# ZENGXH/DMM_Net

Hardware: AMD Instinct MI355X
Metric: frames/sec (cost+match layer) at N=50 proposals, M=10 templates, 255x255 (higher is better)
Workload: dtype f32

## Files before the change

### dmm_net_amd/csrc/dmm_api.hip

```cpp
#include <limits.h>
#include <stdlib.h>

#include <atomic>

#include "dmm_launchers.h"
#include "dmm_solve.h"

namespace dmm {
static thread_local int g_last_hip_error = 0;
void set_last_hip_error(int e) { g_last_hip_error = e; }
static std::atomic<long long> g_launches{0};
void note_launch() { g_launches.fetch_add(1, std::memory_order_relaxed); }

static constexpr int kOptDefaults[DMM_OPT_COUNT] = {
     -1,       8,    -1,   0,
     0,      8192,         512,  512,
     1,           3,             320000,     2,
     128,        3,              512,  1,
     65,    1,           4,     1,
     -1,        1,    -1,  1,
};
static std::atomic<int> g_opts[DMM_OPT_COUNT] = {
    {kOptDefaults[0]},  {kOptDefaults[1]},  {kOptDefaults[2]},  {kOptDefaults[3]},  {kOptDefaults[4]},
    {kOptDefaults[5]},  {kOptDefaults[6]},  {kOptDefaults[7]},  {kOptDefaults[8]},  {kOptDefaults[9]},
    {kOptDefaults[10]}, {kOptDefaults[11]}, {kOptDefaults[12]}, {kOptDefaults[13]}, {kOptDefaults[14]},
    {kOptDefaults[15]}, {kOptDefaults[16]}, {kOptDefaults[17]}, {kOptDefaults[18]}, {kOptDefaults[19]},
    {kOptDefaults[20]}, {kOptDefaults[21]}, {kOptDefaults[22]}, {kOptDefaults[23]},
};
static_assert(DMM_OPT_COUNT == 24, "kOptDefaults / g_opts list every option");
int opt(int key) { return g_opts[key].load(std::memory_order_relaxed); }

static inline size_t align_up(size_t v, size_t a) { return (v + a - 1) / a * a; }

struct Workspace {
    int32_t *inter, *area_p, *area_t;
    float *featn_p, *featn_t, *cosv, *sim, *Rb;
    float *wide;
    size_t bytes;
};

static bool wide_shape(int N, int M) {
    const int Pp = N > M ? N : M + 1;
    return M > DMM_MAX_TEMPLATES || Pp > DMM_MAX_PROPOSALS || opt(DMM_OPT_FORCE_WIDE) == 1;
}

static Workspace carve(void *base, int B, int N, int M, int D) {
    const int Pp = N > M ? N : M + 1;
    Workspace w;
    size_t off = 0;
    auto take = [&](size_t n) {
        void *p = base ? (void *)((char *)base + off) : nullptr;
        off += align_up(n, 256);
        return p;
    };
    w.inter = (int32_t *)take(sizeof(int32_t) * ((size_t)B * M * N + (size_t)B * N + (size_t)B * M));
    w.area_p = w.inter ? w.inter + (size_t)B * M * N : nullptr;
    w.area_t = w.area_p ? w.area_p + (size_t)B * N : nullptr;
    w.featn_p = (float *)take(sizeof(float) * (size_t)B * N * D);
    w.featn_t = (float *)take(sizeof(float) * (size_t)B * M * D);
    w.cosv = (float *)take(sizeof(float) * (size_t)B * M * N);
    w.sim = (float *)take(sizeof(float) * (size_t)B * M * N);
    w.Rb = (float *)take(sizeof(float) * (size_t)B * M * Pp);
    w.wide = nullptr;
    if (wide_shape(N, M))
        w.wide = (float *)take(sizeof(float) * (size_t)B * wide_scratch_floats(M, Pp));
    w.bytes = off;
    return w;
}

static float *or_ws(float *out, float *ws) { return out ? out : ws; }

static Front ws_front(const Workspace &w, const void *masks_p, const void *masks_t, int dtype, int64_t sp_b, int64_t sp_n,
                      int64_t st_b, int64_t st_m, const float *feat_p, const float *feat_t, int B, int N, int M, int HW, int D,
                      const int32_t *n_valid, const int32_t *m_valid) {
    Front f{};
    f.masks_p = masks_p; f.masks_t = masks_t; f.dtype = dtype;
    f.sp_b = sp_b; f.sp_n = sp_n; f.st_b = st_b; f.st_m = st_m;
    f.feat_p = feat_p; f.feat_t = feat_t;
    f.B = B; f.N = N; f.M = M; f.HW = HW; f.D = D;
    f.n_valid = n_valid; f.m_valid = m_valid;
    f.cos = w.cosv;
    f.inter = w.inter; f.area_p = w.area_p; f.area_t = w.area_t;
    f.table_words = (size_t)B * M * N + (size_t)B * N + (size_t)B * M;
    f.featn_p = w.featn_p; f.featn_t = w.featn_t;
    return f;
}
static Front packed_front(const Workspace &w, const uint64_t *packed_p, int64_t pk_b, int64_t pk_n, const uint64_t *packed_t,
                          const float *feat_p, const float *feat_t, int B, int N, int M, int HW, int D,
                          const int32_t *n_valid, const int32_t *m_valid) {
    const int64_t wd = dmm_pack_words(HW);
    Front f = ws_front(w, packed_p, packed_t, DMM_PACKED1, pk_b, pk_n, (int64_t)M * wd, wd, feat_p, feat_t, B, N, M, HW, D,
                       n_valid, m_valid);
    f.ragged_lanes = true;
    return f;
}
}

extern "C" int dmm_abi_version(void) { return DMM_ABI_VERSION; }

extern "C" int dmm_set_option(int option, int value) {
    if (option < 0 || option >= DMM_OPT_COUNT) return DMM_ERR_BAD_ARG;
    switch (option) {
        case DMM_OPT_FEAT_BWD_FRAME: if (value < -1 || value > 2) return DMM_ERR_BAD_ARG; break;
        case DMM_OPT_COST_KERNEL: case DMM_OPT_SOLVER_KERNEL: case DMM_OPT_MIX_SHARED:
            if (value < -1 || value > 1) return DMM_ERR_BAD_ARG; break;
        case DMM_OPT_MIX_XCD: if (value < 0 || value > 7) return DMM_ERR_BAD_ARG; break;
        case DMM_OPT_FORCE_WIDE: case DMM_OPT_COSINE_KERNEL: case DMM_OPT_COST_XCD:
        case DMM_OPT_NMS_WAVE: case DMM_OPT_SMALL_FUSED: case DMM_OPT_MIX_SHARED_LOCKSTEP:
            if (value < 0 || value > 1) return DMM_ERR_BAD_ARG; break;
        case DMM_OPT_MIX_ALIGN: if (value != 16 && value != 32 && value != 64 && value != 128) return DMM_ERR_BAD_ARG; break;
        case DMM_OPT_MIX_NT: if (value < 0 || value > 3) return DMM_ERR_BAD_ARG; break;
        case DMM_OPT_COST_WGS: case DMM_OPT_COST_SMALL_WGS: case DMM_OPT_COST_TL_WGS: case DMM_OPT_MIX_WGS:
        case DMM_OPT_MIX_STEPQ: case DMM_OPT_GEMM_TUNE: case DMM_OPT_COS_ROWS_MIN_N: case DMM_OPT_MIX_SHARED_STEPS:
            if (value < 1) return DMM_ERR_BAD_ARG; break;
        default: if (value < 0) return DMM_ERR_BAD_ARG; break;
    }
    dmm::g_opts[option].store(value, std::memory_order_relaxed);
    return DMM_OK;
}

extern "C" int dmm_get_option(int option) {
    return (option < 0 || option >= DMM_OPT_COUNT) ? INT_MIN : dmm::opt(option);
}

extern "C" int dmm_reset_options(void) {
    for (int k = 0; k < DMM_OPT_COUNT; ++k) dmm::g_opts[k].store(dmm::kOptDefaults[k], std::memory_order_relaxed);
    return DMM_OK;
}

extern "C" const char *dmm_status_string(int status) {
    switch (status) {
        case DMM_OK: return "ok";
        case DMM_ERR_BAD_ARG: return "bad argument";
        case DMM_ERR_UNSUPPORTED: return "shape outside the compiled kernel envelope";
        case DMM_ERR_LAUNCH: return "HIP launch/runtime error (see dmm_last_hip_error)";
        case DMM_ERR_WORKSPACE: return "workspace too small";
        default: return "unknown status";
    }
}

extern "C" int dmm_last_hip_error(void) { return dmm::g_last_hip_error; }

extern "C" long long dmm_launch_count(void) { return dmm::g_launches.load(std::memory_order_relaxed); }

#define DMM_STR_(x) #x
#define DMM_STR(x) DMM_STR_(x)
extern "C" const char *dmm_build_info(void) { return "libdmm_match gfx950 (CDNA4, wave64) abi " DMM_STR(DMM_ABI_VERSION); }

extern "C" size_t dmm_workspace_bytes(int B, int N, int M, int D) {
    if (B <= 0 || N <= 0 || M <= 0 || D < 0) return 0;
    return dmm::carve(nullptr, B, N, M, D).bytes;
}

extern "C" int dmm_match_forward(const void *masks_p, const void *masks_t, int mask_dtype, const float *feat_p,
                                 const float *feat_t, const float *score_p, int B, int N, int M, int HW, int D,
                                 int64_t sp_b, int64_t sp_n, int64_t st_b, int64_t st_m, const int32_t *n_valid,
                                 const int32_t *m_valid, float score_weight, int max_iter, int proj_iter, float lr,
                                 int is_test, float *full_outmask, float *match_score, float *det_score,
                                 float *sim_out, float *R_out, float *Rb_out, int32_t *iters_out, void *workspace,
                                 size_t workspace_bytes, dmm_stream_t stream) {
    return dmm_match_forward_ws(masks_p, masks_t, mask_dtype, feat_p, feat_t, score_p, B, N, M, HW, D, sp_b, sp_n, st_b, st_m,
                                n_valid, m_valid, score_weight, max_iter, proj_iter, lr, is_test, full_outmask, match_score,
                                det_score, sim_out, R_out, Rb_out, iters_out, workspace, workspace_bytes, nullptr, stream);
}

extern "C" int dmm_match_forward_ws(const void *masks_p, const void *masks_t, int mask_dtype, const float *feat_p,
                                    const float *feat_t, const float *score_p, int B, int N, int M, int HW, int D,
                                    int64_t sp_b, int64_t sp_n, int64_t st_b, int64_t st_m, const int32_t *n_valid,
                                    const int32_t *m_valid, float score_weight, int max_iter, int proj_iter, float lr,
                                    int is_test, float *full_outmask, float *match_score, float *det_score,
                                    float *sim_out, float *R_out, float *Rb_out, int32_t *iters_out, void *workspace,
                                    size_t workspace_bytes, int *ws_state, dmm_stream_t stream) {
    const bool tables_zero = ws_state && *ws_state == DMM_WS_TABLES_ZERO;
    if (ws_state) *ws_state = DMM_WS_UNKNOWN;
    bool go;
    int rc = dmm::one_call_check(B, N, M, HW, D, masks_p && masks_t && feat_p && feat_t && score_p && full_outmask &&
                                 match_score && det_score && workspace, &go);
    if (!go) return rc;
    if (!dmm::soft_planes(mask_dtype)) return DMM_ERR_BAD_ARG;
    const dmm::Workspace w = dmm::carve(workspace, B, N, M, D);
    if (workspace_bytes < w.bytes) return DMM_ERR_WORKSPACE;
    const dmm::SolveIn in{w.cosv, w.inter, w.area_p, w.area_t, score_p, B, N, M, n_valid, m_valid};
    const dmm::SolveOut out{dmm::or_ws(sim_out, w.sim), R_out, dmm::or_ws(Rb_out, w.Rb), match_score, det_score, iters_out,
                            nullptr};
    const dmm::RelaxParams prm{max_iter, proj_iter, lr};
    if (dmm::wide_shape(N, M)) {
        if (!w.wide || B > 65535) return DMM_ERR_UNSUPPORTED;
// ... 120 lines not shown
```

### dmm_net_amd/csrc/dmm_gemm.hip

```cpp
#include <hipblaslt/hipblaslt.h>

#include <initializer_list>
#include <map>
#include <mutex>
#include <tuple>
#include <vector>

#include "dmm_common.h"

namespace dmm {
namespace {

struct GemmPlan {
    hipblasLtMatmulDesc_t desc = nullptr;
    hipblasLtMatrixLayout_t a = nullptr, b = nullptr, c = nullptr, d = nullptr;
    hipblasLtMatmulAlgo_t algo;
    size_t workspace = 0;
    bool ok = false;
    std::vector<hipblasLtMatmulHeuristicResult_t> candidates;
};

constexpr int kTuneCandidates = 24, kTuneRuns = 8;

std::mutex g_mu;
std::map<int, hipblasLtHandle_t> g_handles;
hipblasLtHandle_t handle_of(int dev) {
    auto it = g_handles.find(dev);
    if (it != g_handles.end()) return it->second;
    hipblasLtHandle_t h = nullptr;
    if (hipblasLtCreate(&h) != HIPBLAS_STATUS_SUCCESS) return nullptr;
    g_handles[dev] = h;
    return h;
}
std::map<std::tuple<int, int64_t, int, int, int, int, int>, GemmPlan> g_plans;

void release_plan(GemmPlan &p) {
    if (p.desc) hipblasLtMatmulDescDestroy(p.desc);
    for (hipblasLtMatrixLayout_t l : {p.a, p.b, p.c, p.d})
        if (l) hipblasLtMatrixLayoutDestroy(l);
    p = GemmPlan();
}

#define DMM_LT_TRY(expr)                                    \
    do {                                                    \
        if ((expr) != HIPBLAS_STATUS_SUCCESS) return false; \
    } while (0)

bool build_plan(hipblasLtHandle_t g_handle, GemmPlan &p, int64_t rows, int cin, int cout, bool relu, bool residual, size_t ws_limit) {
    const hipDataType bf16 = HIP_R_16BF;
    DMM_LT_TRY(hipblasLtMatmulDescCreate(&p.desc, HIPBLAS_COMPUTE_32F, HIP_R_32F));
    const hipblasOperation_t op_n = HIPBLAS_OP_N;
    DMM_LT_TRY(hipblasLtMatmulDescSetAttribute(p.desc, HIPBLASLT_MATMUL_DESC_TRANSA, &op_n, sizeof(op_n)));
    DMM_LT_TRY(hipblasLtMatmulDescSetAttribute(p.desc, HIPBLASLT_MATMUL_DESC_TRANSB, &op_n, sizeof(op_n)));
    const hipblasLtEpilogue_t epi = relu ? HIPBLASLT_EPILOGUE_RELU_BIAS : HIPBLASLT_EPILOGUE_BIAS;
    DMM_LT_TRY(hipblasLtMatmulDescSetAttribute(p.desc, HIPBLASLT_MATMUL_DESC_EPILOGUE, &epi, sizeof(epi)));
    const int32_t bias_type = (int32_t)HIP_R_32F;
    DMM_LT_TRY(hipblasLtMatmulDescSetAttribute(p.desc, HIPBLASLT_MATMUL_DESC_BIAS_DATA_TYPE, &bias_type, sizeof(bias_type)));
    DMM_LT_TRY(hipblasLtMatrixLayoutCreate(&p.a, bf16, cout, cin, cout));
    DMM_LT_TRY(hipblasLtMatrixLayoutCreate(&p.b, bf16, cin, rows, cin));
    DMM_LT_TRY(hipblasLtMatrixLayoutCreate(&p.c, bf16, cout, rows, cout));
    DMM_LT_TRY(hipblasLtMatrixLayoutCreate(&p.d, bf16, cout, rows, cout));
    hipblasLtMatmulPreference_t pref = nullptr;
    DMM_LT_TRY(hipblasLtMatmulPreferenceCreate(&pref));
    const uint64_t ws = ws_limit;
    hipblasLtMatmulPreferenceSetAttribute(pref, HIPBLASLT_MATMUL_PREF_MAX_WORKSPACE_BYTES, &ws, sizeof(ws));
    const void *dummy = (const void *)0x1000;
    hipblasLtMatmulDescSetAttribute(p.desc, HIPBLASLT_MATMUL_DESC_BIAS_POINTER, &dummy, sizeof(dummy));
    const int want = [] {
        const int v = dmm::opt(DMM_OPT_GEMM_TUNE);
        return v < 1 ? 1 : (v > kTuneCandidates ? kTuneCandidates : v);
    }();
    hipblasLtMatmulHeuristicResult_t res[kTuneCandidates];
    int found = 0;
    const hipblasStatus_t st = hipblasLtMatmulAlgoGetHeuristic(g_handle, p.desc, p.a, p.b, residual ? p.c : p.d, p.d, pref,
                                                               want, res, &found);
    hipblasLtMatmulPreferenceDestroy(pref);
    if (st != HIPBLAS_STATUS_SUCCESS || found < 1) return false;
    p.algo = res[0].algo;
    p.workspace = res[0].workspaceSize;
    p.ok = true;
    for (int i = 0; i < found; ++i)
        if (res[i].state == HIPBLAS_STATUS_SUCCESS && res[i].workspaceSize <= ws_limit) p.candidates.push_back(res[i]);
    if (p.candidates.size() < 2) p.candidates.clear();
    return true;
}

void tune_plan(hipblasLtHandle_t g_handle, GemmPlan &p, const void *x, const void *w, const void *residual, void *y, void *workspace,
               size_t workspace_bytes, hipStream_t stream) {
    std::vector<hipblasLtMatmulHeuristicResult_t> cand;
    cand.swap(p.candidates);
    hipEvent_t e0 = nullptr, e1 = nullptr;
    if (hipEventCreate(&e0) != hipSuccess) return;
    if (hipEventCreate(&e1) != hipSuccess) { (void)hipEventDestroy(e0); return; }
    const float alpha = 1.0f, beta = residual ? 1.0f : 0.0f;
    float best = 0.0f;
    int best_i = -1;
    for (size_t i = 0; i < cand.size(); ++i) {
        bool ok = true;
        for (int r = 0; r < kTuneRuns + 1 && ok; ++r) {
            if (r == 1 && hipEventRecord(e0, stream) != hipSuccess) ok = false;
            ok = ok && hipblasLtMatmul(g_handle, p.desc, &alpha, w, p.a, x, p.b, &beta, residual ? residual : y,
                                       residual ? p.c : p.d, y, p.d, &cand[i].algo, workspace, workspace_bytes,
                                       stream) == HIPBLAS_STATUS_SUCCESS;
        }
        float ms = 0.0f;
        if (!ok || hipEventRecord(e1, stream) != hipSuccess || hipEventSynchronize(e1) != hipSuccess ||
            hipEventElapsedTime(&ms, e0, e1) != hipSuccess) {
            (void)hipGetLastError();
            continue;
        }
        if (best_i < 0 || ms < best) { best = ms; best_i = (int)i; }
    }
    (void)hipEventDestroy(e0);
    (void)hipEventDestroy(e1);
    if (best_i >= 0) {
        p.algo = cand[best_i].algo;
        p.workspace = cand[best_i].workspaceSize;
    }
}

}
}

extern "C" int dmm_conv1x1_bf16(const void *x, const void *w, const float *bias, const void *residual, int64_t rows,
                                int cin, int cout, int relu, void *y, void *workspace, size_t workspace_bytes,
                                dmm_stream_t stream) {
    if (rows < 0 || cin <= 0 || cout <= 0) return DMM_ERR_BAD_ARG;
    if (rows == 0) return DMM_OK;
    if (!x || !w || !bias || !y) return DMM_ERR_BAD_ARG;
    int dev = 0;
    DMM_HIP_TRY(hipGetDevice(&dev));
    const size_t avail = workspace ? workspace_bytes : 0;
    std::lock_guard<std::mutex> lk(dmm::g_mu);
    hipblasLtHandle_t handle = dmm::handle_of(dev);
    if (!handle) return DMM_ERR_LAUNCH;
    auto key = std::make_tuple(dev, rows, cin, cout, relu ? 1 : 0, residual ? 1 : 0, avail ? 1 : 0);
    auto it = dmm::g_plans.find(key);
    if (it == dmm::g_plans.end()) {
        dmm::GemmPlan p;
        if (!dmm::build_plan(handle, p, rows, cin, cout, relu != 0, residual != nullptr, avail)) p.ok = false;
        it = dmm::g_plans.emplace(key, p).first;
    }
    dmm::GemmPlan *plan = &it->second;
    if (plan->ok && plan->workspace > avail) {
        dmm::GemmPlan p;
        if (!dmm::build_plan(handle, p, rows, cin, cout, relu != 0, residual != nullptr, avail)) p.ok = false;
        if (p.ok && p.workspace > avail) p.ok = false;
        if (!p.ok) {
            dmm::release_plan(p);
            return DMM_ERR_UNSUPPORTED;
        }
        dmm::release_plan(*plan);
        *plan = p;
    }
    if (!plan->ok) return DMM_ERR_UNSUPPORTED;
    const void *bp = bias;
    if (hipblasLtMatmulDescSetAttribute(plan->desc, HIPBLASLT_MATMUL_DESC_BIAS_POINTER, &bp, sizeof(bp)) !=
        HIPBLAS_STATUS_SUCCESS)
        return DMM_ERR_LAUNCH;
    if (!plan->candidates.empty()) {
        hipStreamCaptureStatus cs = hipStreamCaptureStatusNone;
        if (hipStreamIsCapturing((hipStream_t)stream, &cs) == hipSuccess && cs == hipStreamCaptureStatusNone)
            dmm::tune_plan(handle, *plan, x, w, residual, y, workspace, workspace_bytes, (hipStream_t)stream);
        else
            (void)hipGetLastError();
    }
    const float alpha = 1.0f, beta = residual ? 1.0f : 0.0f;
    const hipblasStatus_t st =
        hipblasLtMatmul(handle, plan->desc, &alpha, w, plan->a, x, plan->b, &beta, residual ? residual : y,
                        residual ? plan->c : plan->d, y, plan->d, &plan->algo, workspace, workspace_bytes,
                        (hipStream_t)stream);
    if (st != HIPBLAS_STATUS_SUCCESS) {
        dmm::set_last_hip_error((int)st);
        return DMM_ERR_LAUNCH;
    }
    return DMM_OK;
}
```

### dmm_net_amd/csrc/dmm_launchers.h

```cpp
#pragma once
#include "dmm_common.h"

namespace dmm {

int cosine_lanes_launch(const float *feat_t, const float *feat_p, int B, int N, int M, int D, float *cos_out,
                        hipStream_t stream, int32_t *zero_ptr = nullptr, int64_t zero_words = 0,
                        const int32_t *n_valid = nullptr);
int feature_normalize2_launch(const float *in_a, int64_t rows_a, float *out_a, float *norms_a, const float *in_b,
                              int64_t rows_b, float *out_b, float *norms_b, int D, hipStream_t stream,
                              void *zero_ptr = nullptr, size_t zero_bytes = 0);

struct CountArgs {
    const void *masks_p, *masks_t;
    const void *masks_t2;
    int dtype;
    int B, N, M, HW;
    int64_t sp_b, sp_n, st_b, st_m;
    int64_t st2_b, st2_m;
    const int32_t *n_valid, *m_valid;
    int32_t *inter, *area_p, *area_t;
    int32_t *inter2, *area_t2;
};
int iou_counts_launch(const CountArgs &a, bool tables_zeroed, hipStream_t stream);

int mask_mix_bwd_prezeroed(const float *Rb, const void *masks_p, int dtype, const float *dout, int B, int N, int M, int Pp,
                           int HW, int64_t sp_b, int64_t sp_n, const int32_t *n_valid, const int32_t *m_valid, float *dRb,
                           dmm_stream_t stream);

static inline int one_call_check(int B, int N, int M, int HW, int D, bool have_pointers, bool *go) {
    *go = false;
    if (B < 0 || N < 0 || M < 0 || HW < 0 || D < 0) return DMM_ERR_BAD_ARG;
    if (B == 0 || M == 0) return DMM_OK;
    if (N == 0 || !have_pointers) return DMM_ERR_BAD_ARG;
    *go = true;
    return DMM_OK;
}
static inline bool soft_planes(int dtype) { return dtype == DMM_F32 || dtype == DMM_F16 || dtype == DMM_BF16; }

struct Front : CountArgs {
    const float *feat_p, *feat_t;
    int D;
    float *cos;
    size_t table_words;
    float *featn_p, *featn_t;
    bool tables_zero;
    bool ragged_lanes;
    bool dense_tile;
    bool split_norm;
};
int front_small_launch(const Front &f, hipStream_t stream);
int match_front(const Front &f, hipStream_t stream, bool *fused = nullptr);
int match_mix(const float *Rb, const void *masks_p, int dtype, int B, int N, int M, int HW, int64_t sp_b, int64_t sp_n,
              const int32_t *n_valid, const int32_t *m_valid, int is_test, float *full_outmask, dmm_stream_t stream);

}
```

### include/dmm_match.h

```cpp
#ifndef DMM_MATCH_H
#define DMM_MATCH_H

#include <stddef.h>
#include <stdint.h>

#ifdef __cplusplus
extern "C" {
#endif

#define DMM_ABI_VERSION 2

typedef enum dmm_status {
    DMM_OK = 0,
    DMM_ERR_BAD_ARG = 1,
    DMM_ERR_UNSUPPORTED = 2,
    DMM_ERR_LAUNCH = 3,
    DMM_ERR_WORKSPACE = 4
} dmm_status;

typedef enum dmm_dtype {
    DMM_F32 = 0, DMM_F16 = 1, DMM_BF16 = 2,
    DMM_PACKED1 = 3
} dmm_dtype;

typedef void *dmm_stream_t;

#define DMM_API __attribute__((visibility("default")))

#define DMM_MAX_TEMPLATES 32
#define DMM_MAX_PROPOSALS 256

#define DMM_FRAME_TABLE INT64_MIN

typedef enum dmm_option {
    DMM_OPT_COST_KERNEL = 0,
    DMM_OPT_COST_TINY_FRAMES = 1,
    DMM_OPT_SOLVER_KERNEL = 2,
    DMM_OPT_FORCE_WIDE = 3,
    DMM_OPT_COSINE_KERNEL = 4,
    DMM_OPT_COST_WGS = 5,
    DMM_OPT_COST_SMALL_WGS = 6,
    DMM_OPT_COST_TL_WGS = 7,
    DMM_OPT_COST_XCD = 8,
    DMM_OPT_MIX_XCD = 9,
    DMM_OPT_MIX_WGS = 10,
    DMM_OPT_MIX_STEPQ = 11,
    DMM_OPT_MIX_ALIGN = 12,
    DMM_OPT_MIX_NT = 13,
    DMM_OPT_SOLVER_HELPER_MAX = 14,
    DMM_OPT_NMS_WAVE = 15,
    DMM_OPT_COS_ROWS_MIN_N = 16,
    DMM_OPT_GEMM_TUNE = 17,
    DMM_OPT_PACK_VARIANT = 18,
    DMM_OPT_SMALL_FUSED = 19,
    DMM_OPT_MIX_SHARED = 20,
    DMM_OPT_MIX_SHARED_STEPS = 21,
    DMM_OPT_FEAT_BWD_FRAME = 22,
    DMM_OPT_MIX_SHARED_LOCKSTEP = 23,
    DMM_OPT_COUNT = 24
} dmm_option;
DMM_API int dmm_set_option(int option, int value);
DMM_API int dmm_get_option(int option);
DMM_API int dmm_reset_options(void);

DMM_API int dmm_abi_version(void);
DMM_API const char *dmm_status_string(int status);
DMM_API int dmm_last_hip_error(void);
DMM_API const char *dmm_build_info(void);
DMM_API long long dmm_launch_count(void);

DMM_API int dmm_iou_counts(const void *masks_p, const void *masks_t, int dtype, int B, int N, int M, int HW,
                   int64_t sp_b, int64_t sp_n, int64_t st_b, int64_t st_m,
                   const int32_t *n_valid, const int32_t *m_valid,
                   int32_t *inter , int32_t *area_p , int32_t *area_t ,
                   dmm_stream_t stream);

DMM_API int64_t dmm_pack_words(int HW);
DMM_API int dmm_pack_masks(const void *masks, int dtype, int64_t planes, int HW, int64_t plane_stride,
                           uint64_t *packed, int64_t packed_stride, dmm_stream_t stream);

DMM_API int dmm_iou_counts_dual(const void *masks_p, const void *masks_t, const void *masks_t2, int dtype, int B,
                                int N, int M, int HW, int64_t sp_b, int64_t sp_n, int64_t st_b, int64_t st_m,
                                int64_t st2_b, int64_t st2_m, const int32_t *n_valid, const int32_t *m_valid,
                                int32_t *inter, int32_t *area_p, int32_t *area_t, int32_t *inter2, int32_t *area_t2,
                                dmm_stream_t stream);

DMM_API int dmm_iou_counts_frames(const void *const *masks_p_frames, const void *masks_t, int dtype, int B, int N,
                                  int M, int HW, int64_t sp_n, int64_t st_b, int64_t st_m, const int32_t *n_valid,
                                  const int32_t *m_valid, int32_t *inter, int32_t *area_p, int32_t *area_t,
                                  dmm_stream_t stream);
DMM_API int dmm_iou_counts_dual_frames(const void *const *masks_p_frames, const void *masks_t, const void *masks_t2,
                                       int dtype, int B, int N, int M, int HW, int64_t sp_n, int64_t st_b,
                                       int64_t st_m, int64_t st2_b, int64_t st2_m, const int32_t *n_valid,
                                       const int32_t *m_valid, int32_t *inter, int32_t *area_p, int32_t *area_t,
                                       int32_t *inter2, int32_t *area_t2, dmm_stream_t stream);
DMM_API int dmm_mask_mix_frames(const float *Rb, const void *const *masks_p_frames, int dtype, int B, int N, int M,
                                int Pp, int HW, int64_t sp_n, const int32_t *n_valid, const int32_t *m_valid,
                                float *out, int64_t so_b, int64_t so_m, dmm_stream_t stream);
DMM_API int dmm_mask_mix_bwd_frames(const float *Rb, const void *const *masks_p_frames, int dtype, const float *dout,
                                    int B, int N, int M, int Pp, int HW, int64_t sp_n, const int32_t *n_valid,
                                    const int32_t *m_valid, float *dRb, dmm_stream_t stream);

DMM_API int dmm_feature_normalize_f32(const float *in, int64_t rows, int D, float *out ,
                              float *norms , dmm_stream_t stream);

DMM_API int dmm_cosine_features_f32(const float *feat_t , const float *feat_p , int B, int N,
                                    int M, int D, float *cos_out , dmm_stream_t stream);

DMM_API int dmm_feature_sim_bwd_f32(const float *dsim , const float *cos , const float *gt,
                                    const float *d_loss, float score_weight, const float *feat_t, const float *feat_p,
                                    const float *featn_t, const float *featn_p, const float *norm_t, const float *norm_p,
                                    int B, int N, int M, int D, const int32_t *n_valid, const int32_t *m_valid,
                                    float *g_feat_t , float *g_feat_p , dmm_stream_t stream);

DMM_API int dmm_cosine_f32(const float *featn_t , const float *featn_p , int B, int N, int M,
                           int D, const int32_t *n_valid, const int32_t *m_valid, float *cos_out ,
                           dmm_stream_t stream);

DMM_API int dmm_relax_match_f32(const float *cos_in, const int32_t *inter, const int32_t *area_p,
                                const int32_t *area_t, const float *score_p , int B, int N, int M,
                                const int32_t *n_valid, const int32_t *m_valid,
                                float score_weight, int max_iter, int proj_iter, float lr, int is_test,
                                float *sim_out, float *R_out, float *Rb_out,
                                float *match_score, float *det_score, int32_t *iters_out, float *X_final,
                                dmm_stream_t stream);

DMM_API size_t dmm_relax_any_scratch_bytes(int B, int N, int M);
DMM_API int dmm_relax_match_any_f32(const float *cos_in, const int32_t *inter, const int32_t *area_p,
                                    const int32_t *area_t, const float *score_p, int B, int N, int M,
                                    const int32_t *n_valid, const int32_t *m_valid, float score_weight, int max_iter,
                                    int proj_iter, float lr, int is_test, float *sim_out, float *R_out, float *Rb_out,
                                    float *match_score, float *det_score, int32_t *iters_out, float *X_final,
                                    void *scratch, size_t scratch_bytes, dmm_stream_t stream);

DMM_API int dmm_relax_match_f16s(const float *cos_in, const int32_t *inter, const int32_t *area_p,
                                 const int32_t *area_t, const float *score_p , int B, int N, int M,
                                 const int32_t *n_valid, const int32_t *m_valid,
                                 float score_weight, int max_iter, int proj_iter, float lr, int is_test,
                                 float *sim_out, float *R_out, float *Rb_out,
                                 float *match_score, float *det_score, int32_t *iters_out, float *X_final,
                                 dmm_stream_t stream);

// ... 109 lines not shown
                                    float *cos_out, float *sim_out, float *Rb_out, float *gt_out, void *workspace,
                                    size_t workspace_bytes, void *tape, size_t tape_bytes, int *taped ,
                                    dmm_stream_t stream);
DMM_API size_t dmm_match_train_backward_workspace_bytes(int B, int N, int M, int D, int max_iter, int proj_iter);
DMM_API int dmm_match_train_backward(const void *masks_p, int mask_dtype, const float *feat_p, const float *feat_t,
                                     const float *score_p, const float *cos, const float *sim, const float *Rb,
                                     const float *gt, const float *d_full, const float *d_match_score,
                                     const float *d_det_score, const float *d_loss, int B, int N, int M, int HW, int D,
                                     int64_t sp_b, int64_t sp_n, const int32_t *n_valid, const int32_t *m_valid,
                                     float score_weight, int max_iter, int proj_iter, float lr, int is_test,
                                     float *g_feat_t , float *g_feat_p , void *workspace,
                                     size_t workspace_bytes, const void *tape, const int32_t *iters ,
                                     int taped, dmm_stream_t stream);
DMM_API size_t dmm_match_train_backward_det_workspace_bytes(int B, int N, int M, int D, int max_iter, int proj_iter, int HW);
DMM_API int dmm_match_train_backward_det(const void *masks_p, int mask_dtype, const float *feat_p, const float *feat_t,
                                         const float *score_p, const float *cosv, const float *sim, const float *Rb,
                                         const float *gt, const float *d_full, const float *d_match_score,
                                         const float *d_det_score, const float *d_loss, int B, int N, int M, int HW, int D,
                                         int64_t sp_b, int64_t sp_n, const int32_t *n_valid, const int32_t *m_valid,
                                         float score_weight, int max_iter, int proj_iter, float lr, int is_test,
                                         float *g_feat_t, float *g_feat_p, void *workspace, size_t workspace_bytes,
                                         const void *tape, const int32_t *iters, int taped, dmm_stream_t stream);

DMM_API int dmm_roialign4_mean_nhwc_fwd(const void *const feat[4], int dtype, int B, int C, const int H[4],
                                        const int W[4], const float scale[4], const float *rois, int R, float *out,
                                        dmm_stream_t stream);
DMM_API int dmm_roialign4_mean_fwd(const void *const feat[4], int dtype, int B, int C, const int H[4], const int W[4],
                                   const float scale[4], const float *rois, int R, float *out, dmm_stream_t stream);
DMM_API int dmm_roialign4_mean_bwd(const float *dout, int B, int C, const int H[4], const int W[4],
                                   const float scale[4], const float *rois, int R, float *const dfeat[4],
                                   dmm_stream_t stream);
DMM_API size_t dmm_roialign4_mean_bwd_det_workspace_bytes(int R, const int H[4], const int W[4]);
DMM_API int dmm_roialign4_mean_bwd_det(const float *dout, int B, int C, const int H[4], const int W[4], const float scale[4],
                                       const float *rois, int R, float *const dfeat[4], void *workspace, size_t workspace_bytes,
                                       dmm_stream_t stream);

DMM_API int dmm_paste_masks_f32(const float *prob, int P, int M, const float *boxes, int im_h, int im_w, float thresh,
                                int padding, float *planes, int64_t plane_stride, float *new_boxes,
                                uint64_t *packed ,
                                dmm_stream_t stream);
DMM_API int dmm_nms_f32(const float *boxes, const float *scores, const int32_t *offsets, int images, int max_per_image,
                        float thresh, int max_keep, int32_t *keep, int32_t *keep_count, dmm_stream_t stream);

DMM_API int dmm_proposal_boxes_f32(const float *prob, const float *boxes, const int32_t *counts, int images, int R, int M,
                                   int im_h, int im_w, float thresh, int padding, const int32_t *step, float *tight,
                                   dmm_stream_t stream);
DMM_API int dmm_nms_slots_f32(const float *tight, const float *scores, const int32_t *counts, int images, int R,
                              float thresh, int K, const int32_t *step, int32_t *keep, int32_t *keep_count,
                              dmm_stream_t stream);
DMM_API int dmm_paste_kept_f32(const float *prob, const float *boxes, const float *scores, const float *tight,
                               const int32_t *keep, const int32_t *keep_count, int images, int R, int M, int K, int im_h,
                               int im_w, int padding, const int32_t *step, const int32_t *img_base, float *planes,
                               int64_t plane_stride, uint64_t *packed, float *kept_boxes, float *kept_scores, float *rois,
                               dmm_stream_t stream);

DMM_API int dmm_mask_boxes_f32(const float *masks, int R, int H, int W, int64_t plane_stride, float thresh,
                               float *boxes, int32_t *valid, dmm_stream_t stream);
DMM_API int dmm_merge_labels_f32(const float *masks, int B, int O, int HW, int64_t stride_b, int64_t stride_o,
                                 const int32_t *o_valid, uint8_t *labels, dmm_stream_t stream);

DMM_API int dmm_step_finish_f32(const float *Rb, int Pp, const float *prob, const float *boxes, const int32_t *keep,
                                const int32_t *keep_count, int B, int R, int Mm, int K, int M, int im_h, int im_w,
                                int padding, const int32_t *step, const int32_t *m_valid, const int32_t *commit,
                                const int32_t *o_valid, float *full, float *hist, uint64_t *packed_hist, uint8_t *labels,
                                dmm_stream_t stream);
DMM_API int dmm_step_select_i32(const int32_t *table, const int32_t *step, int n, int32_t *out, dmm_stream_t stream);
DMM_API int dmm_step_advance(int32_t *step, dmm_stream_t stream);
DMM_API int dmm_commit_masks_f32(const float *full, float *hist, const int32_t *commit, int B, int64_t per_video,
                                 dmm_stream_t stream);

DMM_API int dmm_ragged_pad(const void *const *src_table, const int32_t *counts, int B, int P_max, int64_t row_bytes,
                           void *out, dmm_stream_t stream);

DMM_API int dmm_bias_act_bf16(void *x, const float *bias, const void *residual, int64_t rows, int C, int relu,
                              dmm_stream_t stream);

DMM_API int dmm_bias_relu_maxpool_bf16(const void *x, const float *bias, int B, int H, int W, int C, void *y,
                                       dmm_stream_t stream);

DMM_API int dmm_im2col3x3_bf16(const void *x, int B, int H, int W, int C, int stride, void *cols, dmm_stream_t stream);

DMM_API int dmm_conv1x1_bf16(const void *x, const void *w, const float *bias, const void *residual, int64_t rows, int cin,
                             int cout, int relu, void *y, void *workspace, size_t workspace_bytes, dmm_stream_t stream);

DMM_API int dmm_bn_stats_bf16(const void *x, int64_t rows, int C, float *stats, dmm_stream_t stream);
DMM_API int dmm_bn_apply_bf16(const void *x, const void *residual, int64_t rows, int C, const float *stats,
                              const float *weight, const float *bias, float *running_mean, float *running_var,
                              float momentum, float eps, int relu, void *y, float *saved, dmm_stream_t stream);
DMM_API int dmm_bn_bwd_reduce_bf16(const void *dy, const void *x, const void *y, int64_t rows, int C, const float *saved,
                                   const float *weight, const float *bias, int relu, float *sums, dmm_stream_t stream);
DMM_API int dmm_bn_bwd_dx_bf16(const void *dy, const void *x, const void *y, int64_t rows, int C, const float *saved,
                               const float *weight, const float *bias, const float *sums, int relu, void *dx, void *dres,
                               float *dweight, float *dbias, dmm_stream_t stream);
DMM_API int dmm_bn_stats_grouped_bf16(const void *x, int64_t rows, int C, int groups, float *stats, dmm_stream_t stream);
DMM_API int dmm_bn_apply_grouped_bf16(const void *x, const void *residual, int64_t rows, int C, int groups, const float *stats,
                                      const float *weight, const float *bias, float *running_mean, float *running_var,
                                      float momentum, float eps, int relu, void *y, float *saved, dmm_stream_t stream);
DMM_API int dmm_bn_bwd_reduce_grouped_bf16(const void *dy, const void *dy2, const void *x, const void *y, int64_t rows, int C, int groups,
                                           const float *saved, const float *weight, const float *bias, int relu, float *sums,
                                           dmm_stream_t stream);
DMM_API int dmm_bn_bwd_dx_grouped_bf16(const void *dy, const void *dy2, const void *x, const void *y, int64_t rows, int C, int groups,
                                       const float *saved, const float *weight, const float *bias, const float *sums, int relu,
                                       void *dx, void *dres, float *dweight, float *dbias, dmm_stream_t stream);
DMM_API size_t dmm_bn_det_workspace_bytes(int64_t rows, int C, int groups);
DMM_API int dmm_bn_stats_det_grouped_bf16(const void *x, int64_t rows, int C, int groups, void *workspace,
                                          size_t workspace_bytes, dmm_stream_t stream);
DMM_API int dmm_bn_apply_det_grouped_bf16(const void *x, const void *residual, int64_t rows, int C, int groups,
                                          const void *workspace, size_t workspace_bytes, const float *weight, const float *bias,
                                          float *running_mean, float *running_var, float momentum, float eps, int relu, void *y,
                                          float *saved, dmm_stream_t stream);
DMM_API int dmm_bn_bwd_reduce_det_grouped_bf16(const void *dy, const void *dy2, const void *x, const void *y, int64_t rows, int C,
                                               int groups, const float *saved, const float *weight, const float *bias, int relu,
                                               void *workspace, size_t workspace_bytes, dmm_stream_t stream);
DMM_API int dmm_bn_bwd_dx_det_grouped_bf16(const void *dy, const void *dy2, const void *x, const void *y, int64_t rows, int C,
                                           int groups, const float *saved, const float *weight, const float *bias,
                                           const void *workspace, size_t workspace_bytes, int relu, void *dx, void *dres,
                                           float *dweight, float *dbias, dmm_stream_t stream);
DMM_API int dmm_bn_fold_det(const void *workspace, size_t workspace_bytes, int64_t rows, int C, int groups, float *out,
                            dmm_stream_t stream);

DMM_API int dmm_wprep3x3_bf16(const void *table, int n, int64_t tiles, dmm_stream_t stream);
DMM_API int dmm_cast_many_bf16(const void *table, int n, int64_t blocks, dmm_stream_t stream);
DMM_API int dmm_subsample2_bf16(const void *x, int B, int H, int W, int C, void *y, dmm_stream_t stream);
DMM_API int dmm_upsample2_zero_bf16(const void *dy, int B, int H, int W, int C, void *dx, dmm_stream_t stream);
DMM_API size_t dmm_wgrad_workspace_bytes(int64_t rows, int co, int cv);
DMM_API int dmm_wgrad_bf16(const void *dy, const void *x, int64_t rows, int co, int ci, int64_t ldy, int64_t ldx, float *dw,
                           void *workspace, size_t workspace_bytes, dmm_stream_t stream);
DMM_API int dmm_wgrad3x3_bf16(const void *dy, const void *x, int B, int H, int W, int ci, int co, int stride, float *dw,
                              void *workspace, size_t workspace_bytes, dmm_stream_t stream);

DMM_API size_t dmm_conv3x3_workspace_bytes(int B, int H, int W, int ci, int co, int stride);
DMM_API int dmm_conv3x3_bf16(const void *x, const void *w, const void *bias, int B, int H, int W, int ci, int co, int stride,
                             void *y, void *workspace, size_t workspace_bytes, dmm_stream_t stream);

DMM_API int dmm_conv3x3_narrow_bf16(const void *x, const void *w, const void *bias, int B, int H, int W, int ci, int co,
                                    void *y, dmm_stream_t stream);
DMM_API size_t dmm_wgrad3x3_narrow_workspace_bytes(int B, int H, int W, int ci, int co);
DMM_API int dmm_wgrad3x3_narrow_bf16(const void *dy, const void *x, int B, int H, int W, int ci, int co, float *dw,
                                     void *workspace, size_t workspace_bytes, dmm_stream_t stream);

DMM_API int dmm_conv7x7s2_stem_bf16(const void *x, const void *w, const void *bias, int B, int H, int W, void *y,
                                    dmm_stream_t stream);
DMM_API size_t dmm_wgrad7x7s2_stem_workspace_bytes(int B, int H, int W);
DMM_API int dmm_wgrad7x7s2_stem_bf16(const void *dy, const void *x, int B, int H, int W, float *dw, void *workspace,
                                     size_t workspace_bytes, dmm_stream_t stream);

DMM_API int dmm_graph_nodes_to_kernels(void *graph, int flags, int *n_memset, int *n_memcpy, int *n_left);

DMM_API int dmm_mask_pyramid_f32(const float *prev_mask, const float *y_mask, const float *init_pred, int64_t sb_prev,
                                 int64_t so_prev, int64_t sb_y, int64_t so_y, int64_t sb_init, int64_t so_init, int B, int n_obj,
                                 int H, int W, float *out5, float *out4, float *out3, float *out2, dmm_stream_t stream);
DMM_API int dmm_clstm_gates_f32(const float *pre0, const float *pre1, const float *pre2, int64_t sb0, int64_t sb1, int64_t sb2,
                                const float *masks, int64_t sb_masks, const float *w_mask, const float *cell_prev, int B,
                                int hidden_size, int h, int w, float *hidden, float *cell, float *hidden_copy, int64_t sb_copy,
                                dmm_stream_t stream);
DMM_API size_t dmm_clstm_gates_bwd_workspace_bytes(int B, int hidden_size, int h, int w);
DMM_API int dmm_clstm_gates_bwd_f32(const float *pre0, const float *pre1, const float *pre2, int64_t sb0, int64_t sb1, int64_t sb2,
                                    const float *masks, int64_t sb_masks, const float *w_mask, const float *cell_prev, int B,
                                    int hidden_size, int h, int w, const float *d_hidden, const float *d_cell, float *d_pre,
                                    float *d_cell_prev, float *d_masks, float *d_w_mask, void *ws, size_t ws_bytes,
                                    dmm_stream_t stream);
DMM_API int dmm_upsample_bilinear_into_f32(const float *src, int64_t sb_src, int B, int C, int h, int w, float *dst,
                                           int64_t sb_dst, int C_dst, int c0, int H, int W, int mode, dmm_stream_t stream);
DMM_API int dmm_refine_finish_f32(const float *logits, int64_t sb_logits, int64_t so_logits, int h, int w, const int *valid,
                                  int B, int O, int n_obj, int H, int W, float *outs, float *mask_hist, dmm_stream_t stream);
DMM_API int dmm_clstm_gates_bf16(const void *pre0, const void *pre1, const void *pre2, int64_t sb0, int64_t sb1, int64_t sb2,
// ... 81 lines not shown
```

Baseline: 298,700.

## Add persistent MFMA streaming kernel for bf16 1x1 convolutions

Adds a custom persistent HIP kernel for bf16 1x1 convolution. It keeps the weight tile resident in LDS, prefetches the next input tile into registers, and uses 32x32x16 bf16 MFMA with a fused bias, residual, ReLU and RNE epilogue. The kernel runs in place of hipBLASLt for large-row shapes that match a short whitelist, aimed at cutting GEMM library overhead and redundant weight loads. This conv path belongs to the backbone and is separate from the cost and match layer being measured, so the benchmark likely does not exercise it.

```diff
diff --git a/dmm_net_amd/csrc/dmm_api.hip b/dmm_net_amd/csrc/dmm_api.hip
--- a/dmm_net_amd/csrc/dmm_api.hip
+++ b/dmm_net_amd/csrc/dmm_api.hip
@@ -19,15 +19,17 @@
      128,        3,              512,  1,
      65,    1,           4,     1,
      -1,        1,    -1,  1,
+     -1,    0,
 };
 static std::atomic<int> g_opts[DMM_OPT_COUNT] = {
     {kOptDefaults[0]},  {kOptDefaults[1]},  {kOptDefaults[2]},  {kOptDefaults[3]},  {kOptDefaults[4]},
     {kOptDefaults[5]},  {kOptDefaults[6]},  {kOptDefaults[7]},  {kOptDefaults[8]},  {kOptDefaults[9]},
     {kOptDefaults[10]}, {kOptDefaults[11]}, {kOptDefaults[12]}, {kOptDefaults[13]}, {kOptDefaults[14]},
     {kOptDefaults[15]}, {kOptDefaults[16]}, {kOptDefaults[17]}, {kOptDefaults[18]}, {kOptDefaults[19]},
-    {kOptDefaults[20]}, {kOptDefaults[21]}, {kOptDefaults[22]}, {kOptDefaults[23]},
+    {kOptDefaults[20]}, {kOptDefaults[21]}, {kOptDefaults[22]}, {kOptDefaults[23]}, {kOptDefaults[24]},
+    {kOptDefaults[25]},
 };
-static_assert(DMM_OPT_COUNT == 24, "kOptDefaults / g_opts list every option");
+static_assert(DMM_OPT_COUNT == 26, "kOptDefaults / g_opts list every option");
 int opt(int key) { return g_opts[key].load(std::memory_order_relaxed); }
 
 static inline size_t align_up(size_t v, size_t a) { return (v + a - 1) / a * a; }
@@ -102,7 +104,7 @@
     if (option < 0 || option >= DMM_OPT_COUNT) return DMM_ERR_BAD_ARG;
     switch (option) {
         case DMM_OPT_FEAT_BWD_FRAME: if (value < -1 || value > 2) return DMM_ERR_BAD_ARG; break;
-        case DMM_OPT_COST_KERNEL: case DMM_OPT_SOLVER_KERNEL: case DMM_OPT_MIX_SHARED:
+        case DMM_OPT_COST_KERNEL: case DMM_OPT_SOLVER_KERNEL: case DMM_OPT_MIX_SHARED: case DMM_OPT_CONV1X1_STREAM:
             if (value < -1 || value > 1) return DMM_ERR_BAD_ARG; break;
         case DMM_OPT_MIX_XCD: if (value < 0 || value > 7) return DMM_ERR_BAD_ARG; break;
         case DMM_OPT_FORCE_WIDE: case DMM_OPT_COSINE_KERNEL: case DMM_OPT_COST_XCD:
diff --git a/dmm_net_amd/csrc/dmm_gemm.hip b/dmm_net_amd/csrc/dmm_gemm.hip
--- a/dmm_net_amd/csrc/dmm_gemm.hip
+++ b/dmm_net_amd/csrc/dmm_gemm.hip
@@ -7,6 +7,7 @@
 #include <vector>
 
 #include "dmm_common.h"
+#include "dmm_launchers.h"
 
 namespace dmm {
 namespace {
@@ -128,6 +129,9 @@
     if (rows < 0 || cin <= 0 || cout <= 0) return DMM_ERR_BAD_ARG;
     if (rows == 0) return DMM_OK;
     if (!x || !w || !bias || !y) return DMM_ERR_BAD_ARG;
+    if (dmm::conv1x1_stream_takes(rows, cin, cout, residual != nullptr) &&
+        (((uintptr_t)x | (uintptr_t)w | (uintptr_t)bias | (uintptr_t)residual | (uintptr_t)y) & 15u) == 0)
+        return dmm::conv1x1_stream_launch(x, w, bias, residual, rows, cin, cout, relu, y, (hipStream_t)stream);
     int dev = 0;
     DMM_HIP_TRY(hipGetDevice(&dev));
     const size_t avail = workspace ? workspace_bytes : 0;
diff --git a/dmm_net_amd/csrc/dmm_gemm_stream.hip b/dmm_net_amd/csrc/dmm_gemm_stream.hip
--- /dev/null
+++ b/dmm_net_amd/csrc/dmm_gemm_stream.hip
@@ -0,0 +1,260 @@
+#include "dmm_common.h"
+#include "dmm_launchers.h"
+
+namespace dmm {
+
+typedef __bf16 bf16x8s __attribute__((ext_vector_type(8)));
+typedef float f32x16s __attribute__((ext_vector_type(16)));
+typedef float f32x4s __attribute__((ext_vector_type(4)));
+typedef uint32_t u32x4s __attribute__((ext_vector_type(4)));
+
+constexpr int kStreamCUs = 256;
+constexpr int kStreamLdsPerCU = 160 * 1024;
+
+struct StreamGeom {
+    int64_t rows, tiles, per;
+    int cout, relu, ranges, nc;
+};
+
+__device__ __forceinline__ uint32_t stream_bf16_rne(float v) {
+    const uint32_t u = __float_as_uint(v);
+    if ((u & 0x7fffffffu) > 0x7f800000u) return (u >> 16) | 0x40u;
+    return (u + 0x7fffu + ((u >> 16) & 1u)) >> 16;
+}
+__device__ __forceinline__ int stream_lds_at(int r, int p) { return r * 64 + ((p ^ ((r >> 1) & 7)) << 3); }
+__device__ __forceinline__ float bf16_lo(uint32_t u) { return __uint_as_float(u << 16); }
+__device__ __forceinline__ float bf16_hi(uint32_t u) { return __uint_as_float(u & 0xFFFF0000u); }
+
+template <int CIN, int TN, int TM>
+struct StreamShape {
+    static constexpr int W_ELEMS = CIN * TN;
+    static constexpr int OUT_LD = TN + 4;
+    static constexpr int X_BYTES = TM * CIN * 2, O_BYTES = TM * OUT_LD * 4;
+    static constexpr int LDS = W_ELEMS * 2 + (X_BYTES > O_BYTES ? X_BYTES : O_BYTES);
+};
+
+template <int CIN, int TN, int TM, bool RES>
+__global__ __launch_bounds__(256) void conv1x1_stream_kernel(const uint16_t *__restrict__ x, const uint16_t *__restrict__ w,
+                                                             const float *__restrict__ bias, const uint16_t *__restrict__ res,
+                                                             uint16_t *__restrict__ y, StreamGeom g) {
+    typedef StreamShape<CIN, TN, TM> S;
+    constexpr int KC = CIN / 64;
+    constexpr int NI = TN / 64, NJ = TM / 64;
+    constexpr int RB = TM / 32;
+    constexpr int NX = RB * KC;
+    constexpr int PR = TN / 8;
+    constexpr int NO = TM * PR / 256;
+    constexpr int OUT_LD = S::OUT_LD;
+    static_assert(S::LDS <= 160 * 1024 && S::W_ELEMS * 2 <= 64 * 1024, "LDS budget");
+    extern __shared__ __attribute__((aligned(16))) uint16_t stream_lds[];
+    uint16_t *sW = stream_lds, *sX = stream_lds + S::W_ELEMS;
+    float *sO = reinterpret_cast<float *>(sX);
+
+    const int t = threadIdx.x, lane = t & 63, wave = t >> 6;
+    const int r = lane & 31, h = lane >> 5;
+    const int wco = wave & 1, wpx = wave >> 1;
+
+    int id = blockIdx.x;
+    if (g.nc > 1) id = (id & 7) * (int)(gridDim.x >> 3) + (id >> 3);
+    if (id >= g.ranges * g.nc) return;
+    const int f = id / g.nc, co0 = (id - f * g.nc) * TN;
+    const int64_t t0 = (int64_t)f * g.per;
+    const int64_t t1 = t0 + g.per < g.tiles ? t0 + g.per : g.tiles;
+
+    const int pc = t & 7, pr = t >> 3;
+    u32x4s rx[NX];
+    auto fetch = [&](int64_t tile) {
+        const int64_t m0 = tile * TM;
+#pragma unroll
+        for (int q = 0; q < NX; ++q) {
+            const int rb = q % RB, ch = q / RB;
+            const int64_t m = m0 + pr + 32 * rb;
+            rx[q] = *reinterpret_cast<const u32x4s *>(x + (m < g.rows ? m * CIN : (int64_t)0) + ch * 64 + pc * 8);
+        }
+    };
+    if (t0 < t1) fetch(t0);
+
+    {
+        constexpr int TASKS = (TN / 8) * (CIN / 8);
+#pragma unroll
+        for (int u = 0; u < (TASKS + 255) / 256; ++u) {
+            const int e = t + 256 * u;
+            if (e < TASKS) {
+                const int cb = e % (TN / 8), kb = e / (TN / 8);
+                u32x4s v[8];
+#pragma unroll
+                for (int i = 0; i < 8; ++i)
+                    v[i] = *reinterpret_cast<const u32x4s *>(w + (int64_t)(kb * 8 + i) * g.cout + co0 + cb * 8);
+#pragma unroll
+                for (int j = 0; j < 8; ++j) {
+                    u32x4s o;
+#pragma unroll
+                    for (int m = 0; m < 4; ++m) {
+                        const uint32_t a = v[2 * m][j >> 1], b = v[2 * m + 1][j >> 1];
+                        o[m] = (j & 1) ? ((a >> 16) | (b & 0xFFFF0000u)) : ((a & 0xFFFFu) | (b << 16));
+                    }
+                    *reinterpret_cast<u32x4s *>(sW + (kb >> 3) * (TN * 64) + stream_lds_at(cb * 8 + j, kb & 7)) = o;
+                }
+            }
+        }
+    }
+
+    for (int64_t tile = t0; tile < t1; ++tile) {
+        const int64_t m0 = tile * TM;
+        u32x4s rr[RES ? NO : 1];
+        if constexpr (RES) {
+#pragma unroll
+            for (int n = 0; n < NO; ++n) {
+                const int idx = t + 256 * n, pl = idx / PR, p8 = idx % PR;
+                const int64_t m = m0 + pl;
+                rr[n] = *reinterpret_cast<const u32x4s *>(res + (m < g.rows ? m * g.cout : (int64_t)0) + co0 + 8 * p8);
+            }
+        }
+#pragma unroll
+        for (int q = 0; q < NX; ++q) {
+            const int rb = q % RB, ch = q / RB;
+            *reinterpret_cast<u32x4s *>(sX + ch * (TM * 64) + stream_lds_at(pr + 32 * rb, pc)) = rx[q];
+        }
+        if (tile + 1 < t1) fetch(tile + 1);
+        __syncthreads();
+
+        f32x16s acc[NI][NJ];
+#pragma unroll
+        for (int i = 0; i < NI; ++i)
+#pragma unroll
+            for (int j = 0; j < NJ; ++j)
+#pragma unroll
+                for (int k = 0; k < 16; ++k) acc[i][j][k] = 0.0f;
+#pragma unroll
+        for (int kk = 0; kk < CIN / 16; ++kk) {
+            const int ch = kk >> 2, p = 2 * (kk & 3) + h;
+            bf16x8s fa[NI], fb[NJ];
+#pragma unroll
+            for (int i = 0; i < NI; ++i)
+                fa[i] = *reinterpret_cast<const bf16x8s *>(sW + ch * (TN * 64) + stream_lds_at(wco * (32 * NI) + i * 32 + r, p));
+#pragma unroll
+            for (int j = 0; j < NJ; ++j)
+                fb[j] = *reinterpret_cast<const bf16x8s *>(sX + ch * (TM * 64) + stream_lds_at(wpx * (32 * NJ) + j * 32 + r, p));
+#pragma unroll
+            for (int i = 0; i < NI; ++i)
+#pragma unroll
+                for (int j = 0; j < NJ; ++j) acc[i][j] = __builtin_amdgcn_mfma_f32_32x32x16_bf16(fa[i], fb[j], acc[i][j], 0, 0, 0);
+        }
+        __syncthreads();
+
+#pragma unroll
+        for (int i = 0; i < NI; ++i)
+#pragma unroll
+            for (int g4 = 0; g4 < 4; ++g4) {
+                const int cl = wco * (32 * NI) + i * 32 + 8 * g4 + 4 * h;
+                const f32x4s bv = *reinterpret_cast<const f32x4s *>(bias + co0 + cl);
+#pragma unroll
+                for (int j = 0; j < NJ; ++j) {
+                    const int pl = wpx * (32 * NJ) + j * 32 + r;
+                    const f32x4s v = {acc[i][j][4 * g4] + bv[0], acc[i][j][4 * g4 + 1] + bv[1], acc[i][j][4 * g4 + 2] + bv[2],
+                                      acc[i][j][4 * g4 + 3] + bv[3]};
+                    *reinterpret_cast<f32x4s *>(sO + pl * OUT_LD + cl) = v;
+                }
+            }
+        __syncthreads();
+#pragma unroll
+        for (int n = 0; n < NO; ++n) {
+            const int idx = t + 256 * n, pl = idx / PR, p8 = idx % PR;
+            const int64_t m = m0 + pl;
+            const f32x4s a = *reinterpret_cast<const f32x4s *>(sO + pl * OUT_LD + 8 * p8);
+            const f32x4s b = *reinterpret_cast<const f32x4s *>(sO + pl * OUT_LD + 8 * p8 + 4);
+            float v[8] = {a[0], a[1], a[2], a[3], b[0], b[1], b[2], b[3]};
+            if constexpr (RES) {
+#pragma unroll
+                for (int k = 0; k < 4; ++k) {
+                    v[2 * k] = v[2 * k] + bf16_lo(rr[n][k]);
+                    v[2 * k + 1] = v[2 * k + 1] + bf16_hi(rr[n][k]);
+                }
+            }
+            if (g.relu) {
+#pragma unroll
+                for (int k = 0; k < 8; ++k) v[k] = v[k] > 0.0f ? v[k] : 0.0f;
+            }
+            u32x4s o;
+#pragma unroll
+            for (int k = 0; k < 4; ++k) o[k] = stream_bf16_rne(v[2 * k]) | (stream_bf16_rne(v[2 * k + 1]) << 16);
+            if (m < g.rows) *reinterpret_cast<u32x4s *>(y + m * g.cout + co0 + 8 * p8) = o;
+        }
+        __syncthreads();
+    }
+}
+
+template <int CIN, int TN, int TM, bool RES>
+int stream_launch_as(const void *x, const void *w, const float *bias, const void *residual, int64_t rows, int cout, int relu,
+                     void *y, hipStream_t stream) {
+    typedef StreamShape<CIN, TN, TM> S;
+    StreamGeom g;
+    g.rows = rows;
+    g.cout = cout;
+    g.relu = relu ? 1 : 0;
+    g.nc = cout / TN;
+    g.tiles = (rows + TM - 1) / TM;
+    const int per_cu = kStreamLdsPerCU / S::LDS < 4 ? kStreamLdsPerCU / S::LDS : 4;
+    const int want = opt(DMM_OPT_CONV1X1_STREAM_WGS);
+    int64_t ranges = (want > 0 ? want : kStreamCUs * per_cu) / g.nc;
+    if (ranges < 1) ranges = 1;
+    if (ranges > g.tiles) ranges = g.tiles;
+    g.per = (g.tiles + ranges - 1) / ranges;
+    g.ranges = (int)((g.tiles + g.per - 1) / g.per);
+    unsigned grid = (unsigned)(g.ranges * g.nc);
+    if (g.nc > 1) grid = (grid + 7u) & ~7u;
+    auto kernel = conv1x1_stream_kernel<CIN, TN, TM, RES>;
+    if (S::LDS > 64 * 1024)
+        DMM_HIP_TRY(hipFuncSetAttribute((const void *)kernel, hipFuncAttributeMaxDynamicSharedMemorySize, S::LDS));
+    hipLaunchKernelGGL(kernel, dim3(grid), dim3(256), S::LDS, stream, (const uint16_t *)x, (const uint16_t *)w, bias,
+                       (const uint16_t *)residual, (uint16_t *)y, g);
+    return check_launch();
+}
+
+template <int CIN, int TN, int TM>
+int stream_launch_res(const void *x, const void *w, const float *bias, const void *residual, int64_t rows, int cout, int relu,
+                      void *y, hipStream_t stream) {
+    return residual ? stream_launch_as<CIN, TN, TM, true>(x, w, bias, residual, rows, cout, relu, y, stream)
+                    : stream_launch_as<CIN, TN, TM, false>(x, w, bias, residual, rows, cout, relu, y, stream);
+}
+
+struct StreamClass { int cin, cout, residual; };
+constexpr StreamClass kStreamClasses[] = {
+    {256, 64, 0},
+    {64, 64, 0},
+};
+constexpr int64_t kStreamMinRows = 32768;
+
+bool conv1x1_stream_envelope(int64_t rows, int cin, int cout) {
+    return rows >= 1 && (cin == 64 || cin == 128 || cin == 256 || cin == 512) && cout >= 64 && cout <= 512 && cout % 64 == 0;
+}
+
+bool conv1x1_stream_takes(int64_t rows, int cin, int cout, bool residual) {
+    const int pin = opt(DMM_OPT_CONV1X1_STREAM);
+    if (pin == 0 || !conv1x1_stream_envelope(rows, cin, cout)) return false;
+    if (pin == 1) return true;
+    if (rows < kStreamMinRows) return false;
+    for (const StreamClass &c : kStreamClasses)
+        if (c.cin == cin && c.cout == cout && (c.residual < 0 || c.residual == (residual ? 1 : 0))) return true;
+    return false;
+}
+
+int conv1x1_stream_launch(const void *x, const void *w, const float *bias, const void *residual, int64_t rows, int cin, int cout,
+                          int relu, void *y, hipStream_t stream) {
+    const bool wide = cout % 128 == 0 && cin <= 256;
+#define DMM_STREAM_GO(CIN, TN, TM) return stream_launch_res<CIN, TN, TM>(x, w, bias, residual, rows, cout, relu, y, stream)
+    switch (cin) {
+        case 64: if (wide) DMM_STREAM_GO(64, 128, 64); else DMM_STREAM_GO(64, 64, 128);
+        case 128: if (wide) DMM_STREAM_GO(128, 128, 64); else DMM_STREAM_GO(128, 64, 64);
+        case 256: if (wide) DMM_STREAM_GO(256, 128, 64); else DMM_STREAM_GO(256, 64, 64);
+        case 512: DMM_STREAM_GO(512, 64, 64);
+        default: return DMM_ERR_UNSUPPORTED;
+    }
+#undef DMM_STREAM_GO
+}
+
+}
+
+extern "C" int dmm_conv1x1_stream_takes(int64_t rows, int cin, int cout, int residual) {
+    return dmm::conv1x1_stream_takes(rows, cin, cout, residual != 0) ? 1 : 0;
+}
diff --git a/dmm_net_amd/csrc/dmm_launchers.h b/dmm_net_amd/csrc/dmm_launchers.h
--- a/dmm_net_amd/csrc/dmm_launchers.h
+++ b/dmm_net_amd/csrc/dmm_launchers.h
@@ -50,6 +50,10 @@
 };
 int front_small_launch(const Front &f, hipStream_t stream);
 int match_front(const Front &f, hipStream_t stream, bool *fused = nullptr);
+bool conv1x1_stream_envelope(int64_t rows, int cin, int cout);
+bool conv1x1_stream_takes(int64_t rows, int cin, int cout, bool residual);
+int conv1x1_stream_launch(const void *x, const void *w, const float *bias, const void *residual, int64_t rows, int cin, int cout,
+                          int relu, void *y, hipStream_t stream);
 int match_mix(const float *Rb, const void *masks_p, int dtype, int B, int N, int M, int HW, int64_t sp_b, int64_t sp_n,
               const int32_t *n_valid, const int32_t *m_valid, int is_test, float *full_outmask, dmm_stream_t stream);
 
diff --git a/include/dmm_match.h b/include/dmm_match.h
--- a/include/dmm_match.h
+++ b/include/dmm_match.h
@@ -57,7 +57,9 @@
     DMM_OPT_MIX_SHARED_STEPS = 21,
     DMM_OPT_FEAT_BWD_FRAME = 22,
     DMM_OPT_MIX_SHARED_LOCKSTEP = 23,
-    DMM_OPT_COUNT = 24
+    DMM_OPT_CONV1X1_STREAM = 24,
+    DMM_OPT_CONV1X1_STREAM_WGS = 25,
+    DMM_OPT_COUNT = 26
 } dmm_option;
 DMM_API int dmm_set_option(int option, int value);
 DMM_API int dmm_get_option(int option);
@@ -333,6 +335,7 @@
 
 DMM_API int dmm_conv1x1_bf16(const void *x, const void *w, const float *bias, const void *residual, int64_t rows, int cin,
                              int cout, int relu, void *y, void *workspace, size_t workspace_bytes, dmm_stream_t stream);
+DMM_API int dmm_conv1x1_stream_takes(int64_t rows, int cin, int cout, int residual);
 
 DMM_API int dmm_bn_stats_bf16(const void *x, int64_t rows, int C, float *stats, dmm_stream_t stream);
 DMM_API int dmm_bn_apply_bf16(const void *x, const void *residual, int64_t rows, int C, const float *stats,
```

Result: no change. 298,400 (-0.1%).
